# EnricoMiccoli/nodal

Hardware: AMD Instinct MI355X
Metric: circuits_per_sec (higher is better)
Workload: dtype f64; 1 GPU; cfg3: grid(1000) 1e6 nodes, sparse CSR path; n=999999, nnz=4995995, parallelism=one GPU

## Files before the change

nodal_amd/csrc/knobs.h:

```cpp
#pragma once
#include <stdint.h>
#include <stdlib.h>

#include <optional>

namespace knob {

struct Present {
    const char *name;
    bool now() const { return getenv(name) != nullptr; }
};
struct OnUnless0 {
    const char *name;
    bool now() const { const char *e = getenv(name); return !(e && atoi(e) == 0); }
};
struct OffUnlessNon0 {
    const char *name;
    bool now() const { const char *e = getenv(name); return e && atoi(e) != 0; }
};
struct OnIfSet0 {
    const char *name;
    bool now() const { const char *e = getenv(name); return e != nullptr && atoi(e) == 0; }
};
struct Level {
// ... 71 lines not shown
inline constexpr Int64 LOWDEG_MIN{"NODAL_LOWDEG_MIN", 32};
inline constexpr Present SPARSE_FORCE_DIRECT{"NODAL_SPARSE_FORCE_DIRECT"};
inline constexpr Present SPARSE_CHILD_DIRECT{"NODAL_SPARSE_CHILD_DIRECT"};
inline constexpr OnUnless0 SAGG{"NODAL_SAGG"};
inline constexpr OnUnless0 SA_REUSE{"NODAL_SA_REUSE"};
inline constexpr OnUnless0 SA_FORK{"NODAL_SA_FORK"};
inline constexpr Double SA_SPREAD{"NODAL_SA_SPREAD", 16.0};
inline constexpr Double SA_SHARE{"NODAL_SA_SHARE", 0.9};
inline constexpr IntIfSet SA_MIS{"NODAL_SA_MIS"};
inline constexpr Text SA_OMEGA_P{"NODAL_SA_OMEGA_P"};
inline constexpr Double SA_PADSLACK{"NODAL_SA_PADSLACK", 1.3};
inline constexpr OnUnless0 SA_D16{"NODAL_SA_D16"};
inline constexpr Int SA_GG{"NODAL_SA_GG", 40};
inline constexpr Int64 SA_GCAP{"NODAL_SA_GCAP", 16384};
inline constexpr Int SA_GSEG{"NODAL_SA_GSEG", 4};
inline constexpr Text SA_NU{"NODAL_SA_NU"};
inline constexpr Int SA_KCYCLE{"NODAL_SA_KCYCLE", 1};
inline constexpr Int SA_KLEVELS{"NODAL_SA_KLEVELS", 1};
inline constexpr OnUnless0 SA_KFREEZE{"NODAL_SA_KFREEZE"};
inline constexpr OnUnless0 SA_FUSE_DIR{"NODAL_SA_FUSE_DIR"};
inline constexpr OffUnlessNon0 SA_GRAPH{"NODAL_SA_GRAPH"};
inline constexpr Text SA_FOLD_POST{"NODAL_SA_FOLD_POST"};
inline constexpr OffUnlessNon0 SA_FOLD_CHECK{"NODAL_SA_FOLD_CHECK"};
inline constexpr OnUnless0 SA_TAIL_DENSE{"NODAL_SA_TAIL_DENSE"};
inline constexpr OffUnlessNon0 SA_TAIL_CHECK{"NODAL_SA_TAIL_CHECK"};
inline constexpr Int SA_TAIL_NU{"NODAL_SA_TAIL_NU", 3};
inline constexpr Present TAIL_PROBE{"NODAL_TAIL_PROBE"};
inline constexpr IntIfSet AMG_PASSES0{"NODAL_AMG_PASSES0"};
inline constexpr IntIfSet AMG_PASSES1{"NODAL_AMG_PASSES1"};
inline constexpr IntIfSet AMG_SWEEPS0{"NODAL_AMG_SWEEPS0"};
// ... 32 lines not shown
```

nodal_amd/csrc/sagg.hip:

```cpp
#include <hip/hip_ext.h>

#include <atomic>
#include <type_traits>

#include "group.h"

int grounded_flags(nodal_ctx *h, uint8_t *flags_dev);

namespace {

using grp::TB;
constexpr int PW = 4;
constexpr int ACAP = 64;
constexpr int RCAP = 96;
constexpr int RCAP_SMALL = 512;
constexpr int RCAP_SMALL_ROWS = 16384;
inline int rcap_for(int64_t nc) { return nc <= RCAP_SMALL_ROWS ? RCAP_SMALL : RCAP; }
constexpr int W0_MAX = 32;
constexpr int COARSEST = 64;
constexpr int MAX_LEVELS = 12;
constexpr int MIS_ROUNDS = 6;
constexpr int TAIL_MAX_N = 1024;
constexpr int TAIL_LEVELS = 6;
constexpr int TAIL_LDS_BUDGET = 150 * 1024;
// ... 99 lines not shown
    bool dense_coarsest = true;
    DevBuf tail_stamps, tail_image, apcol, apval, aplen, bstat;
    DevBuf tail_op;
    bool tail_dense = false;
    DevBuf mvec;
    hipEvent_t ev_copy = nullptr;
    hipStream_t aux = nullptr;
    hipEvent_t ev_fork = nullptr, ev_join = nullptr, ev_flags = nullptr;
    bool aux_pending = false;
    bool aux_tried = false;
    bool want_flags = false;
    int flags_levels = 0;
    DevBuf stats, coarse_inv, mis_t, mis_m, mis_flag, mis_id, agg1, keys, rstart, cursor, lists;
    TailDesc td;
    uint64_t *host_stats = nullptr;
    bool sym_valid = false;
    uint64_t sym_epoch = 0;
    int64_t sym_n = 0, sym_nnz = 0;
    bool sym_general = false, sym_check = false;
    int32_t sym_floating = 0;
    hipGraph_t it_graph = nullptr;
    hipGraphExec_t it_exec = nullptr;
    uint64_t it_key = 0;
    bool refreshed = false;
    int last_iters = 0;
    int hint_iters = 0;
    int64_t hint_n = 0, hint_nnz = 0;
    int mblock_iters = 0;
    int64_t mblock_n = 0;
    unsigned long long sym_stats[MAX_LEVELS * ST_COUNT] = {0};
// ... 26 lines not shown
        tail_op.release();
        mvec.release();
        tail_stamps.release();
        bstat.release();
        apcol.release();
        apval.release();
        aplen.release();
        DevBuf *b[] = {&stats, &coarse_inv, &mis_t, &mis_m, &mis_flag, &mis_id, &agg1, &keys, &rstart, &cursor, &lists};
        for (DevBuf *x : b) x->release();
        if (host_stats) (void)hipHostFree(host_stats);
    }
};


constexpr int BSTAT_MAX = 65536;
__global__ __launch_bounds__(1024) void reduce_bstat(int nblocks, const uint32_t *__restrict__ bstat,
                                                     unsigned long long *__restrict__ stats, int slot_max,
                                                     int slot_sum) {
    __shared__ unsigned int s_max;
    __shared__ unsigned long long s_sum;
    if (threadIdx.x == 0) { s_max = 0; s_sum = 0; }
    __syncthreads();
    unsigned int m = 0;
    unsigned long long t = 0;
    for (int i = threadIdx.x; i < nblocks; i += 1024) {
        m = max(m, bstat[i]);
        t += bstat[BSTAT_MAX + i];
    }
    atomicMax(&s_max, m);
    atomicAdd(&s_sum, t);
    __syncthreads();
    if (threadIdx.x == 0) {
        if (slot_max >= 0) stats[slot_max] = s_max;
        if (slot_sum >= 0) stats[slot_sum] = s_sum;
    }
}

__global__ __launch_bounds__(TB) void row_stats(int64_t n, const int32_t *__restrict__ indptr,
                                                const int32_t *__restrict__ indices,
                                                const double *__restrict__ data, double share, double spread,
                                                bool general, unsigned long long *__restrict__ stats,
                                                uint32_t *__restrict__ bstat) {
    int32_t mlen = 0;
    uint32_t graded = 0, bad = 0, far = 0;
    for (int64_t i = (int64_t)xcd_block() * TB + threadIdx.x; i < n; i += (int64_t)gridDim.x * TB) {
        const int32_t e0 = indptr[i], e1 = indptr[i + 1];
        mlen = max(mlen, e1 - e0);
        double d = 0.0, mx = 0.0, mn = 1e300;
        for (int32_t e = e0; e < e1; ++e) {
            const double v = data[e];
            const int64_t dc = (int64_t)indices[e] - i;
            if (dc > 32767 || dc < -32767) far = 1;
            if (indices[e] == (int32_t)i) d = v;
            else if (v != 0.0) {
                mx = fmax(mx, fabs(v));
                mn = fmin(mn, fabs(v));
                if (v > 0.0 && !general) bad = 1;
            }
        }
        if (!(d > 0.0)) bad = 1;
        graded += (d > 0.0 && (mx > share * d || mx > spread * mn)) ? 1u : 0u;
    }
    __shared__ unsigned int s_len, s_graded, s_bad;
    if (threadIdx.x == 0) s_len = s_graded = s_bad = 0;
    __syncthreads();
    atomicMax(&s_len, (unsigned)mlen);
    if (graded) atomicAdd(&s_graded, graded);
    if (bad) atomicOr(&s_bad, 1u);
    if (far) atomicOr(&s_bad, 2u);
    __syncthreads();
    if (threadIdx.x == 0) {
        bstat[blockIdx.x] = s_len;
        bstat[BSTAT_MAX + blockIdx.x] = s_graded;
        if (s_bad & 1u) atomicOr(&stats[ST_BADDIAG], 1ull);
        if (s_bad & 2u) stats[ST_FARCOL] = 1ull;
    }
}

__global__ __launch_bounds__(TB) void csr_to_ell(int64_t n, int64_t ld, const int32_t *__restrict__ indptr,
                                                 const int32_t *__restrict__ indices,
                                                 const double *__restrict__ data, int32_t *__restrict__ col,
                                                 double *__restrict__ val, float *__restrict__ valf,
                                                 int32_t *__restrict__ len, double *__restrict__ dinv, int32_t wpad,
                                                 int16_t *__restrict__ dcol) {
    for (int64_t i = (int64_t)xcd_block() * TB + threadIdx.x; i < n; i += (int64_t)gridDim.x * TB) {
        const int32_t e0 = indptr[i], e1 = indptr[i + 1];
        double d = 1.0;
        for (int32_t e = e0; e < e1; ++e) {
            const int32_t c = indices[e];
            const double v = data[e];
            col[(int64_t)(e - e0) * ld + i] = c;
            if (dcol) dcol[(int64_t)(e - e0) * ld + i] = (int16_t)(c - (int32_t)i);
            val[(int64_t)(e - e0) * ld + i] = v;
            valf[(int64_t)(e - e0) * ld + i] = (float)v;
            if (c == (int32_t)i) d = v;
        }
        for (int32_t s = e1 - e0; s < wpad; ++s) {
            col[(int64_t)s * ld + i] = (int32_t)i;
            if (dcol) dcol[(int64_t)s * ld + i] = 0;
// ... 188 lines not shown
                for (int u = 0; u < NB; ++u) {
                    if (s0 + u >= l || c[u] == (int32_t)i || aj[u] < 0) continue;
                    if (w[u] > bw) { bw = w[u]; a = aj[u]; }
                }
            };
            if (l <= 5) batch(std::integral_constant<int, 5>{}, 0);
            else for (int32_t s0 = 0; s0 < l; s0 += 8) batch(std::integral_constant<int, 8>{}, s0);
            if (a < 0) stats[ST_UNASSIGNED] = 1;
        }
        agg[i] = a;
    }
}

__global__ __launch_bounds__(TB) void build_P(Ell A, const double *__restrict__ dinv,
                                              const int32_t *__restrict__ agg, int32_t *__restrict__ pcol,
                                              double *__restrict__ pval, float *__restrict__ pvalf, double omega_p) {
    for (int64_t i = (int64_t)xcd_block() * TB + threadIdx.x; i < A.n; i += (int64_t)gridDim.x * TB) {
        int32_t c[PW];
        double v[PW];
#pragma unroll
        for (int k = 0; k < PW; ++k) { c[k] = -1; v[k] = 0.0; }
        const int32_t own = agg[i];
        c[0] = own;
        v[0] = 1.0;
        const double wd = omega_p * dinv[i];
        const int32_t l = A.len[i];
        for (int32_t s = 0; s < l; ++s) {
            const int32_t J = agg[A.col[(int64_t)s * A.ld + i]];
            const double t = -wd * A.val[(int64_t)s * A.ld + i];
            bool placed = false;
#pragma unroll
// ... 30 lines not shown
                                             uint64_t *__restrict__ keys) {
    for (int64_t i = (int64_t)xcd_block() * TB + threadIdx.x; i < n; i += (int64_t)gridDim.x * TB) {
#pragma unroll
        for (int k = 0; k < PW; ++k) {
            const int32_t J = pcol[(int64_t)k * ld + i];
            if (J >= 0) keys[rstart[J] + place[(int64_t)k * ld + i]] = ((uint64_t)i << 2) | (uint64_t)k;
        }
    }
}
__global__ __launch_bounds__(TB) void r_to_ell(int64_t nc, int64_t rld, const uint32_t *__restrict__ rstart,
                                               const uint64_t *__restrict__ keys, int64_t ld,
                                               const double *__restrict__ pval, int32_t *__restrict__ rcol,
                                               double *__restrict__ rval, float *__restrict__ rvalf,
                                               int32_t *__restrict__ rlen,
                                               unsigned long long *__restrict__ stats, uint32_t *__restrict__ bstat,
                                               uint32_t rcap) {
    uint32_t mlen = 0;
    const int sub = threadIdx.x & 7;
    const int64_t rows_per_pass = (int64_t)gridDim.x * (TB / 8);
    for (int64_t I = (int64_t)xcd_block() * (TB / 8) + threadIdx.x / 8; I < nc; I += rows_per_pass) {
        const uint32_t s0 = rstart[I];
        uint32_t l = rstart[I + 1] - s0;
        mlen = l > mlen ? l : mlen;
        if (l > rcap) l = rcap;
        const uint32_t upto = nc <= 4096 ? rcap : ((l + 7u) & ~7u);
        for (uint32_t t = sub; t < upto; t += 8) {
            const int64_t at = ((int64_t)(t >> 3) * rld + I) * 8 + (t & 7);
            if (t < l) {
                const uint64_t key = keys[s0 + t];
                const int64_t i = (int64_t)(key >> 2);
                const double v = pval[(int64_t)(key & 3) * ld + i];
// ... 8 lines not shown
        }
        if (sub == 0) rlen[I] = (int32_t)l;
    }
    if (mlen > rcap) atomicOr(&stats[ST_OVERFLOW], 2ull);
    __shared__ unsigned int s_max;
    if (threadIdx.x == 0) s_max = 0;
    __syncthreads();
#pragma unroll
    for (int off = 32; off > 0; off >>= 1) {
        const uint32_t o = __shfl_down(mlen, off, 64);
        mlen = o > mlen ? o : mlen;
    }
    if ((threadIdx.x & 63) == 0) atomicMax(&s_max, mlen);
    __syncthreads();
    if (threadIdx.x == 0) {
        bstat[blockIdx.x] = s_max;
        bstat[BSTAT_MAX + blockIdx.x] = 0;
    }
}

__global__ __launch_bounds__(TB) void r_refresh(int64_t nc, int64_t rld, const int32_t *__restrict__ rlen,
                                                const int32_t *__restrict__ rcol, int64_t ld,
                                                const int32_t *__restrict__ pcol, const double *__restrict__ pval,
                                                double *__restrict__ rval, float *__restrict__ rvalf) {
    const int sub = threadIdx.x & 7;
    const int64_t rows_per_pass = (int64_t)gridDim.x * (TB / 8);
    for (int64_t I = (int64_t)xcd_block() * (TB / 8) + threadIdx.x / 8; I < nc; I += rows_per_pass) {
        const int32_t l = rlen[I];
        for (int32_t t = sub; t < l; t += 8) {
            const int64_t at = ((int64_t)(t >> 3) * rld + I) * 8 + (t & 7);
            const int64_t i = rcol[at];
            double v = 0.0;
// ... 278 lines not shown
    }
    for (int p = lane + np; p < np + 72; p += 64) lJ[p] = -1;
    __syncthreads();
    return np;
}

template <bool NUMERIC>
__global__ __launch_bounds__(64) void galerkin(int64_t ld, const int32_t *__restrict__ apcol,
                                               const double *__restrict__ apval, const int32_t *__restrict__ aplen,
                                               int64_t nc, int64_t rld, const int32_t *__restrict__ rcol,
                                               const double *__restrict__ rval, const int32_t *__restrict__ rlen,
                                               int64_t cld, int32_t *__restrict__ ccol, double *__restrict__ cval,
                                               float *__restrict__ cvalf,
                                               int32_t *__restrict__ clen, double *__restrict__ cdinv,
                                               unsigned long long *__restrict__ stats, uint32_t *__restrict__ bstat,
                                               int G, int pcap, int maxseg) {
    extern __shared__ __attribute__((aligned(16))) char gsm[];
    int32_t *set = reinterpret_cast<int32_t *>(gsm);
    double *lV = reinterpret_cast<double *>(gsm + 1024);
    int32_t *lJ = reinterpret_cast<int32_t *>(lV + pcap);
    const int lane = threadIdx.x;
    uint32_t my_max = 0, my_nnz = 0, my_flags = 0;
    for (int64_t I = blockIdx.x; I < nc; I += gridDim.x) {
        const int rl = rlen[I];
        const int ngroups = (rl + G - 1) / G;
        int np = 0;
        int total = 0;
        int32_t myJ = 0x7fffffff;
        if constexpr (NUMERIC) {
            total = clen[I];
            if (lane < total) myJ = ccol[(int64_t)lane * cld + I];
// ... 82 lines not shown
            cval[(int64_t)lane * cld + I] = acc;
            cvalf[(int64_t)lane * cld + I] = (float)acc;
            if (myJ == (int32_t)I) {
                if (!(acc > 0.0)) my_flags |= 4u;
                cdinv[I] = acc > 0.0 ? 1.0 / acc : 1.0;
            }
        }
        if (lane == 0) {
            clen[I] = total;
            my_max = (uint32_t)total > my_max ? (uint32_t)total : my_max;
            my_nnz += (uint32_t)total;
        }
        __syncthreads();
    }
    if (lane == 0) {
        bstat[blockIdx.x] = my_max;
        bstat[BSTAT_MAX + blockIdx.x] = my_nnz;
    }
    if (my_flags & 1u) atomicOr(&stats[ST_OVERFLOW], 1ull);
    if (my_flags & 4u) atomicOr(&stats[ST_BADDIAG], 1ull);
}

__global__ __launch_bounds__(256) void coarsest_inverse(Ell A, double *__restrict__ inv,
                                                        unsigned long long *__restrict__ stats) {
    __shared__ double M[COARSEST][2 * COARSEST + 1];
    const int n = (int)A.n;
    for (int t = threadIdx.x; t < n * 2 * n; t += 256) {
        const int r = t / (2 * n), c = t % (2 * n);
        M[r][c] = (c >= n && c - n == r) ? 1.0 : 0.0;
    }
    __syncthreads();
    for (int r = threadIdx.x; r < n; r += 256)
// ... 73 lines not shown

constexpr int SAGG_DECLINED = -3;

int width_class(int maxlen) {
    static const int classes[] = {4, 5, 6, 8, 12, 16, 20, 24, 32};
    for (int c : classes)
        if (maxlen <= c) return c;
    return 0;
}
int choose_wfix(int maxlen, int64_t n, int64_t nnz, int pad_limit) {
    const int c = width_class(maxlen);
    if (c == 0 || c > pad_limit) return 0;
    static const double slack = knob::SA_PADSLACK.now();
    if ((double)c * (double)n <= slack * (double)nnz || n <= 32768) return c;
    return 0;
}

SHierarchy *hierarchy_of(nodal_ctx *h) {
    if (!h->sagg) h->sagg = new SHierarchy();
    return static_cast<SHierarchy *>(h->sagg);
}

struct SolveBufs {
    double *r, *p, *p2, *Ap, *part_rz, *part_zap, *part_rr, *part_pap, *sc;
    cyc_t *z, *x0;
    int g0;
};

template <bool NUMERIC>
int galerkin_product(nodal_ctx *h, SHierarchy *H, int l, hipEvent_t r_ready = nullptr, int phase = 0) {
// ... 27 lines not shown
    }
    if (phase == 1) return NODAL_OK;
    int G = 1024 / apw;
    G = (G < 8 ? 8 : (G > 64 ? 64 : G));
    static const int g_env = knob::SA_GG.now();
    if (g_env >= 8 && g_env <= 64 && apw == 16) G = g_env & ~7;
    const int pcap = G * apw + 72;
    const size_t lds = 1024 + (size_t)pcap * 12;
    static const int64_t gcap = knob::SA_GCAP.now();
    static const int maxseg = knob::SA_GSEG.now();
    const unsigned gg = (unsigned)(nc < gcap ? nc : (gcap < BSTAT_MAX ? gcap : BSTAT_MAX));
    if (r_ready) NODAL_HIP_TRY(h, hipStreamWaitEvent(st, r_ready, 0));
    galerkin<NUMERIC><<<gg, 64, lds, st>>>(
        ld, apcol, apval, aplen, nc, L->rld, L->rcol.as<int32_t>(), L->rval.as<double>(), L->rlen.as<int32_t>(),
        C->ld, C->acol.as<int32_t>(), C->aval.as<double>(), C->avalf.as<float>(), C->alen.as<int32_t>(),
        C->dinv.as<double>(), dstats + (size_t)(l + 1) * ST_COUNT, H->bstat.as<uint32_t>(), G, pcap, maxseg);
    if (!NUMERIC)
        reduce_bstat<<<1, 1024, 0, st>>>((int)gg, H->bstat.as<uint32_t>(), dstats + (size_t)(l + 1) * ST_COUNT,
                                         ST_MAXLEN, ST_NNZ);
    NODAL_HIP_TRY(h, hipGetLastError());
    return NODAL_OK;
}

double omega_p(int level) {
    static double w[2] = {-1.0, -1.0};
    if (w[0] < 0.0) {
        double a = OMEGA_P, b = OMEGA_P_COARSE;
        if (const char *e = knob::SA_OMEGA_P.now()) {
            a = atof(e);
            const char *c = strchr(e, ',');
            b = c ? atof(c + 1) : a;
        }
// ... 72 lines not shown
    static const int mis_rounds = std::min(MIS_ROUNDS, std::max(1, knob::SA_MIS.now().value_or(MIS_ROUNDS)));
    if (n <= MIS_SMALL_MAX && !trace_mis) {
        mis_small<<<1, 1024, 0, st>>>(A, T, M, flag, mis_rounds);
    } else {
        mis_init<<<g, TB, 0, st>>>(n, T);
        for (int r = 0; r < mis_rounds; ++r) {
            mis_max<<<g, TB, 0, st>>>(A, T, M);
            mis_update<<<g, TB, 0, st>>>(A, T, M);
            if (trace_mis) mis_count<<<g, TB, 0, st>>>(n, T, cnt + r + 1);
        }
        mis_flag_roots<<<grid_for(n + 1), TB, 0, st>>>(A, T, flag);
    }
    NODAL_HIP_TRY(h, hipGetLastError());
    NODAL_TRY(scan_exclusive_u32(h, flag, id, n + 1, reinterpret_cast<uint32_t *>(dstats + (size_t)l * ST_COUNT + ST_NC),
                                 scan_tmp));
    NODAL_HIP_TRY(h, hipMemcpyAsync(hs, dstats, (size_t)MAX_LEVELS * ST_COUNT * 8, hipMemcpyDeviceToHost, st));
    unsigned long long hcnt[MIS_ROUNDS + 1] = {0};
    if (trace_mis) NODAL_HIP_TRY(h, hipMemcpyAsync(hcnt, cnt, sizeof hcnt, hipMemcpyDeviceToHost, st));
    if (!H->ev_copy) NODAL_HIP_TRY(h, hipEventCreateWithFlags(&H->ev_copy, hipEventDisableTiming));
    NODAL_HIP_TRY(h, hipEventRecord(H->ev_copy, st));
    NODAL_HIP_TRY(h, L->pcol.reserve((size_t)PW * ld * 4 + 64));
    NODAL_HIP_TRY(h, L->pval.reserve((size_t)PW * ld * 8 + 64));
    NODAL_HIP_TRY(h, L->pvalf.reserve((size_t)PW * ld * 4 + 64));
    assign_near<<<g, TB, 0, st>>>(A, T, flag, id, H->agg1.as<int32_t>());
    assign_far<<<g, TB, 0, st>>>(A, H->agg1.as<int32_t>(), L->agg.as<int32_t>(), dstats + (size_t)l * ST_COUNT);
    build_P<<<g, TB, 0, st>>>(A, L->dinv.as<double>(), L->agg.as<int32_t>(), L->pcol.as<int32_t>(),
                             L->pval.as<double>(), L->pvalf.as<float>(), omega_p(l));
    NODAL_HIP_TRY(h, hipGetLastError());
    NODAL_WAIT_EVENT(h, H->ev_copy, st);
    if (trace_mis) {
        fprintf(stderr, "[sagg] level %d: undecided after each MIS round:", l);
        for (int r = 1; r <= MIS_ROUNDS; ++r) fprintf(stderr, " %llu", hcnt[r]);
        fprintf(stderr, "\n");
    }
    const int64_t nc = (int64_t)(hs[(size_t)l * ST_COUNT + ST_NC] & 0xffffffffull);
    if (l > 0) {
        const unsigned long long *s = hs + (size_t)l * ST_COUNT;
        L->maxlen = (int32_t)s[ST_MAXLEN];
        L->nnz = (int64_t)s[ST_NNZ];
        A.width = L->maxlen;
        if (s[ST_OVERFLOW] || s[ST_BADDIAG] || hs[(size_t)(l - 1) * ST_COUNT + ST_OVERFLOW] ||
            hs[(size_t)(l - 1) * ST_COUNT + ST_UNASSIGNED]) {
            *declined = true;
            return NODAL_OK;
// ... 36 lines not shown
    C->n = nc;
    C->ld = pad64(nc);
    C->width = ACAP;
    C->nc = 0;
    L->rld = C->ld;
    const int rcap = rcap_for(nc);
    NODAL_HIP_TRY(h, L->rcol.reserve((size_t)rcap * C->ld * 4 + 64));
    NODAL_HIP_TRY(h, L->rval.reserve((size_t)rcap * C->ld * 8 + 64));
    NODAL_HIP_TRY(h, L->rvalf.reserve((size_t)rcap * C->ld * 4 + 64));
    NODAL_HIP_TRY(h, L->rlen.reserve((size_t)C->ld * 4 + 64));
    NODAL_HIP_TRY(h, C->acol.reserve((size_t)ACAP * C->ld * 4 + 64));
    NODAL_HIP_TRY(h, C->aval.reserve((size_t)ACAP * C->ld * 8 + 64));
    NODAL_HIP_TRY(h, C->avalf.reserve((size_t)ACAP * C->ld * 4 + 64));
    NODAL_HIP_TRY(h, C->alen.reserve((size_t)C->ld * 4 + 64));
    NODAL_HIP_TRY(h, C->dinv.reserve((size_t)C->ld * 8 + 64));
    if (forked && H->want_flags) {
        if (l == 0) NODAL_HIP_TRY(h, L->gflag.reserve((size_t)n + 64));
        NODAL_HIP_TRY(h, C->gflag.reserve((size_t)C->n + 64));
    }
    {
        const int apw = L->maxlen <= 6 ? 16 : 64;
        NODAL_HIP_TRY(h, H->apcol.reserve((size_t)apw * ld * 4 + 64));
        NODAL_HIP_TRY(h, H->apval.reserve((size_t)apw * ld * 8 + 64));
        NODAL_HIP_TRY(h, H->aplen.reserve((size_t)ld * 4 + 64));
        L->fold = false;
        L->fold_want = fold_wanted(l, n);
        L->wslots = apw;
        if (L->fold_want) {
            NODAL_HIP_TRY(h, L->wcol.reserve((size_t)apw * ld * 4 + 64));
            NODAL_HIP_TRY(h, L->wval.reserve((size_t)apw * ld * 4 + 64));
            NODAL_HIP_TRY(h, L->wlen.reserve((size_t)ld * 4 + 64));
        }
    }
    hipStream_t main_st = h->stream;
// ... 2 lines not shown
        hipStream_t keep;
        ~StreamGuard() { h->stream = keep; }
    } guard{h, main_st};
    if (forked) {
        NODAL_HIP_TRY(h, hipEventRecord(H->ev_fork, main_st));
        NODAL_HIP_TRY(h, hipStreamWaitEvent(H->aux, H->ev_fork, 0));
        H->aux_pending = true;
        NODAL_TRY(galerkin_product<false>(h, H, l, nullptr, 1));
        h->stream = H->aux;
        st = H->aux;
    }
    char *rs = H->rstart.as<char>();
    uint32_t *rstart = reinterpret_cast<uint32_t *>(rs);
    void *scan_tmp2 = rs + a4 + 256;
    uint32_t *place = reinterpret_cast<uint32_t *>(rs + a4 + 256 + scan2);
    NODAL_HIP_TRY(h, hipMemsetAsync(rs, 0, a4 + 256, st));
    r_count<<<g, TB, 0, st>>>(n, ld, L->pcol.as<int32_t>(), rstart, place);
    NODAL_HIP_TRY(h, hipGetLastError());
    NODAL_TRY(scan_exclusive_u32(h, rstart, rstart, nc + 1, nullptr, scan_tmp2));
    uint64_t *keys = H->keys.as<uint64_t>();
    r_fill<<<g, TB, 0, st>>>(n, ld, L->pcol.as<int32_t>(), rstart, place, keys);
    r_sort_short<<<grid_for(nc), TB, 0, st>>>(rstart, keys, nc);
    r_sort_medium<<<(unsigned)(nc < 8192 ? nc : 8192), 64, 0, st>>>(rstart, keys, nc);
    NODAL_HIP_TRY(h, hipGetLastError());

    {
        const unsigned gr = grid_for(nc * 8);
        r_to_ell<<<gr, TB, 0, st>>>(nc, L->rld, rstart, keys, ld, L->pval.as<double>(), L->rcol.as<int32_t>(),
                                   L->rval.as<double>(), L->rvalf.as<float>(), L->rlen.as<int32_t>(),
                                   dstats + (size_t)l * ST_COUNT, H->bstat.as<uint32_t>(), (uint32_t)rcap);
        reduce_bstat<<<1, 1024, 0, st>>>((int)gr, H->bstat.as<uint32_t>(), dstats + (size_t)l * ST_COUNT, ST_MAXR, -1);
    }
    if (forked) {
        NODAL_HIP_TRY(h, hipGetLastError());
        NODAL_HIP_TRY(h, hipEventRecord(H->ev_join, H->aux));
        if (H->want_flags && H->flags_levels == l) {
            if (l == 0) NODAL_TRY(grounded_flags(h, L->gflag.as<uint8_t>()));
            NODAL_HIP_TRY(h, hipMemsetAsync(C->gflag.p, 0, ((size_t)C->n + 63) & ~(size_t)63, st));
            flags_up<<<grid_for(n), TB, 0, st>>>(n, L->agg.as<int32_t>(), L->gflag.as<uint8_t>(), C->gflag.as<uint8_t>());
            NODAL_HIP_TRY(h, hipGetLastError());
            NODAL_HIP_TRY(h, hipEventRecord(H->ev_flags, H->aux));
            H->flags_levels = l + 1;
        }
        h->stream = main_st;
        st = main_st;
    }
    NODAL_TRY(galerkin_product<false>(h, H, l, forked ? H->ev_join : nullptr, forked ? 2 : 0));
    if (forked && H->flags_levels != l + 1) H->aux_pending = false;
    return NODAL_OK;
}

const void *tail_kernel(int slots) {
    return slots <= 8 ? reinterpret_cast<const void *>(k_tail<8>)
// ... 252 lines not shown
}

int sagg_refresh(nodal_ctx *h, SHierarchy *H, const int32_t *indptr0, const int32_t *indices0, const double *data0,
                 bool general, bool *ok) {
    *ok = false;
    hipStream_t st = h->stream;
    unsigned long long *dstats = H->stats.as<unsigned long long>();
    unsigned long long *hs = reinterpret_cast<unsigned long long *>(H->host_stats);
    NODAL_HIP_TRY(h, hipMemsetAsync(dstats, 0, (size_t)MAX_LEVELS * ST_COUNT * 8, st));
    SLevel *L0 = H->pool[0];
    const int64_t n0 = L0->n;
    {
        const unsigned gr = grid_for(n0);
        static const double spread = knob::SA_SPREAD.now();
        static const double share = knob::SA_SHARE.now();
        row_stats<<<gr, TB, 0, st>>>(n0, indptr0, indices0, data0, share, spread, general, dstats, H->bstat.as<uint32_t>());
        reduce_bstat<<<1, 1024, 0, st>>>((int)gr, H->bstat.as<uint32_t>(), dstats, ST_MAXLEN, ST_GRADED);
    }
    csr_to_ell<<<grid_for(n0), TB, 0, st>>>(n0, L0->ld, indptr0, indices0, data0, L0->acol.as<int32_t>(),
                                           L0->aval.as<double>(), L0->avalf.as<float>(),
                                           L0->alen.as<int32_t>(), L0->dinv.as<double>(), L0->wfix,
                                           L0->d16 ? L0->adcol.as<int16_t>() : nullptr);
    NODAL_HIP_TRY(h, hipGetLastError());
    for (int l = 0; l + 1 < H->nlev; ++l) {
        SLevel *L = H->pool[l], *C = H->pool[l + 1];
        Ell A = L->A();
        A.width = L->maxlen;
        build_P<<<grid_for(L->n), TB, 0, st>>>(A, L->dinv.as<double>(), L->agg.as<int32_t>(), L->pcol.as<int32_t>(),
                                              L->pval.as<double>(), L->pvalf.as<float>(), omega_p(l));
        const bool forked = H->aux != nullptr && nodal_extra_streams_ok(h) &&
                            knob::SA_FORK.now();
        hipStream_t rst = st;
        if (forked) {
            NODAL_HIP_TRY(h, hipEventRecord(H->ev_fork, st));
            NODAL_HIP_TRY(h, hipStreamWaitEvent(H->aux, H->ev_fork, 0));
            H->aux_pending = true;
            NODAL_TRY(galerkin_product<true>(h, H, l, nullptr, 1));
            rst = H->aux;
        }
        r_refresh<<<grid_for(C->n * 8), TB, 0, rst>>>(C->n, L->rld, L->rlen.as<int32_t>(), L->rcol.as<int32_t>(), L->ld,
                                                     L->pcol.as<int32_t>(), L->pval.as<double>(), L->rval.as<double>(),
                                                     L->rvalf.as<float>());
        NODAL_HIP_TRY(h, hipGetLastError());
        if (forked) NODAL_HIP_TRY(h, hipEventRecord(H->ev_join, H->aux));
// ... 61 lines not shown
            H->refreshed = true;
            H->ready = true;
            *accepted = true;
            if (trace) fprintf(stderr, "[sagg] symbolic setup kept (struct epoch %llu): values refreshed\n",
                               (unsigned long long)h->struct_epoch);
            return NODAL_OK;
        }
        if (trace) fprintf(stderr, "[sagg] the kept hierarchy does not take the new values: full setup\n");
    }
    H->sym_valid = false;
    H->refreshed = false;
    H->want_flags = check_floating;
    H->flags_levels = 0;
    H->last_iters = 0;
    H->drop_graph();
    NODAL_HIP_TRY(h, H->stats.reserve((size_t)MAX_LEVELS * ST_COUNT * 8 + 64));
    if (!H->host_stats)
        NODAL_HIP_TRY(h, hipHostMalloc(reinterpret_cast<void **>(&H->host_stats), (size_t)MAX_LEVELS * ST_COUNT * 8 + 64));
    unsigned long long *dstats = H->stats.as<unsigned long long>();
    unsigned long long *hs = reinterpret_cast<unsigned long long *>(H->host_stats);
    NODAL_HIP_TRY(h, hipMemsetAsync(dstats, 0, (size_t)MAX_LEVELS * ST_COUNT * 8, st));
    NODAL_HIP_TRY(h, H->bstat.reserve((size_t)2 * BSTAT_MAX * 4 + 64));
    {
        const unsigned gr = grid_for(n0);
        static const double spread = knob::SA_SPREAD.now();
        static const double share = knob::SA_SHARE.now();
        row_stats<<<gr, TB, 0, st>>>(n0, indptr0, indices0, data0, share, spread, general, dstats, H->bstat.as<uint32_t>());
        reduce_bstat<<<1, 1024, 0, st>>>((int)gr, H->bstat.as<uint32_t>(), dstats, ST_MAXLEN, ST_GRADED);
    }
    NODAL_HIP_TRY(h, hipGetLastError());
    NODAL_HIP_TRY(h, hipMemcpyAsync(hs, dstats, ST_COUNT * 8, hipMemcpyDeviceToHost, st));
    NODAL_WAIT_STREAM(h, st);
    const int64_t bar = n0 / 100 < 32 ? (n0 / 100 > 0 ? n0 / 100 : 1) : 32;
    if (hs[ST_MAXLEN] > (unsigned long long)W0_MAX || hs[ST_MAXLEN] == 0 || hs[ST_BADDIAG] ||
        (int64_t)hs[ST_GRADED] >= bar) {
        if (trace)
            fprintf(stderr, "[sagg] declined: longest row %llu, graded nodes %llu (bar %lld), M-matrix %s\n",
                    hs[ST_MAXLEN], hs[ST_GRADED], (long long)bar, hs[ST_BADDIAG] ? "no" : "yes");
        return NODAL_OK;
    }
    SLevel *L0 = H->level(0);
    L0->n = n0;
    L0->ld = pad64(n0);
    L0->maxlen = (int32_t)hs[ST_MAXLEN];
    L0->nnz = nnz0;
    L0->wfix = choose_wfix(L0->maxlen, n0, nnz0, 8);
    L0->width = L0->wfix ? L0->wfix : L0->maxlen;
    NODAL_HIP_TRY(h, L0->acol.reserve((size_t)L0->width * L0->ld * 4 + 64));
    NODAL_HIP_TRY(h, L0->aval.reserve((size_t)L0->width * L0->ld * 8 + 64));
    NODAL_HIP_TRY(h, L0->avalf.reserve((size_t)L0->width * L0->ld * 4 + 64));
    NODAL_HIP_TRY(h, L0->alen.reserve((size_t)L0->ld * 4 + 64));
    NODAL_HIP_TRY(h, L0->dinv.reserve((size_t)L0->ld * 8 + 64));
    static const bool d16_env = knob::SA_D16.now();
    L0->d16 = d16_env && hs[ST_FARCOL] == 0;
    if (L0->d16) NODAL_HIP_TRY(h, L0->adcol.reserve((size_t)L0->width * L0->ld * 2 + 64));
    csr_to_ell<<<grid_for(n0), TB, 0, st>>>(n0, L0->ld, indptr0, indices0, data0, L0->acol.as<int32_t>(),
                                           L0->aval.as<double>(), L0->avalf.as<float>(),
                                           L0->alen.as<int32_t>(), L0->dinv.as<double>(), L0->wfix,
                                           L0->d16 ? L0->adcol.as<int16_t>() : nullptr);
    NODAL_HIP_TRY(h, hipGetLastError());

    int l = 0;
    bool diag_last = false;
    for (;; ++l) {
        SLevel *L = H->level(l);
        if (L->n <= COARSEST && l > 0) break;
        if (l + 1 >= MAX_LEVELS) {
            if (trace) fprintf(stderr, "[sagg] declined: more than %d levels\n", MAX_LEVELS);
            return NODAL_OK;
        }
        bool declined = false, stop = false;
        NODAL_TRY(build_level(h, H, l, hs, &declined, &stop));
        if (declined) {
            if (trace)
                fprintf(stderr, "[sagg] declined at level %d (%lld rows): does not coarsen / over a cap / not positive "
// ... 1 lines not shown
                        l, (long long)L->n, hs[(size_t)l * ST_COUNT + ST_OVERFLOW], hs[(size_t)l * ST_COUNT + ST_BADDIAG],
                        l > 0 ? hs[(size_t)(l - 1) * ST_COUNT + ST_OVERFLOW] : 0ull,
                        l > 0 ? hs[(size_t)(l - 1) * ST_COUNT + ST_UNASSIGNED] : 0ull,
                        l > 0 ? hs[(size_t)(l - 1) * ST_COUNT + ST_MAXR] : 0ull);
            return NODAL_OK;
        }
        if (stop) {
            diag_last = true;
            break;
        }
    }
    H->nlev = l + 1;
    SLevel *last = H->level(l);
    last->fold_want = last->fold = false;
    if (H->nlev < 2) return NODAL_OK;
    NODAL_HIP_TRY(h, hipMemcpyAsync(hs, dstats, (size_t)MAX_LEVELS * ST_COUNT * 8, hipMemcpyDeviceToHost, st));
    if (!H->ev_copy) NODAL_HIP_TRY(h, hipEventCreateWithFlags(&H->ev_copy, hipEventDisableTiming));
    NODAL_HIP_TRY(h, hipEventRecord(H->ev_copy, st));
    if (check_floating) {
        if (H->flags_levels == 0) {
            NODAL_HIP_TRY(h, H->level(0)->gflag.reserve((size_t)n0 + 64));
            NODAL_TRY(grounded_flags(h, H->level(0)->gflag.as<uint8_t>()));
        } else {
            NODAL_HIP_TRY(h, hipStreamWaitEvent(st, H->ev_flags, 0));
            H->aux_pending = false;
        }
        for (int k = H->flags_levels; k + 1 < H->nlev; ++k) {
            SLevel *L = H->pool[k], *C = H->pool[k + 1];
            NODAL_HIP_TRY(h, C->gflag.reserve((size_t)C->n + 64));
            NODAL_HIP_TRY(h, hipMemsetAsync(C->gflag.p, 0, ((size_t)C->n + 63) & ~(size_t)63, st));
            flags_up<<<grid_for(L->n), TB, 0, st>>>(L->n, L->agg.as<int32_t>(), L->gflag.as<uint8_t>(),
                                                   C->gflag.as<uint8_t>());
        }
        NODAL_HIP_TRY(h, hipGetLastError());
    }
    NODAL_WAIT_EVENT(h, H->ev_copy, st);
    for (int k = 0; k < H->nlev; ++k) {
        const unsigned long long *s = hs + (size_t)k * ST_COUNT;
        if (k > 0) {
            H->pool[k]->maxlen = (int32_t)s[ST_MAXLEN];
            H->pool[k]->nnz = (int64_t)s[ST_NNZ];
            H->pool[k]->wfix = choose_wfix(H->pool[k]->maxlen, H->pool[k]->n, H->pool[k]->nnz, APAD);
        }
        if (s[ST_OVERFLOW] || (k > 0 && s[ST_BADDIAG]) || s[ST_UNASSIGNED]) {
            if (trace) fprintf(stderr, "[sagg] declined: level %d over a cap / not positive\n", k);
            return NODAL_OK;
        }
    }
    diag_last = last->maxlen <= 1;
    H->dense_coarsest = !diag_last;
    if (H->dense_coarsest) {
        if (last->n > COARSEST) return NODAL_OK;
        NODAL_HIP_TRY(h, H->coarse_inv.reserve((size_t)last->n * last->n * 8 + 64));
        coarsest_inverse<<<1, 256, 0, st>>>(last->A(), H->coarse_inv.as<double>(),
                                            dstats + (size_t)l * ST_COUNT);
        NODAL_HIP_TRY(h, hipGetLastError());
    }
    for (int k = 0; k < H->nlev; ++k) {
        SLevel *L = H->pool[k];
        NODAL_HIP_TRY(h, L->vec.reserve((size_t)V_COUNT * L->ld * 8 + 256));
        NODAL_HIP_TRY(h, L->part.reserve(5 * DOT_BLOCKS * 8 + 512));
    }
    NODAL_TRY(build_tail(h, H, hs));

    if (!check_floating) {
        NODAL_HIP_TRY(h, hipMemcpyAsync(hs, dstats, (size_t)MAX_LEVELS * ST_COUNT * 8, hipMemcpyDeviceToHost, st));
        NODAL_WAIT_STREAM(h, st);
        if (hs[(size_t)l * ST_COUNT + ST_BADDIAG] & 2ull) return NODAL_OK;
    } else {
        uint32_t *fl = reinterpret_cast<uint32_t *>(dstats + (size_t)(MAX_LEVELS - 1) * ST_COUNT + ST_COUNT - 1);
        if (H->dense_coarsest) last_level_floating<<<1, 64, 0, st>>>(last->A(), last->gflag.as<uint8_t>(), fl);
        else any_unflagged<<<grid_for(last->n), TB, 0, st>>>(last->n, last->gflag.as<uint8_t>(), fl);
        NODAL_HIP_TRY(h, hipGetLastError());
        NODAL_HIP_TRY(h, hipMemcpyAsync(hs, dstats, (size_t)MAX_LEVELS * ST_COUNT * 8, hipMemcpyDeviceToHost, st));
        NODAL_WAIT_STREAM(h, st);
        if (hs[(size_t)l * ST_COUNT + ST_BADDIAG] & 2ull) {
            if (trace) fprintf(stderr, "[sagg] declined: coarsest matrix not positive definite\n");
            return NODAL_OK;
        }
        *floating = hs[(size_t)(MAX_LEVELS - 1) * ST_COUNT + ST_COUNT - 1] != 0 ? 1 : 0;
    }
    if (trace) {
        fprintf(stderr, "[sagg] levels (rows/entries/longest row/padded width):");
        for (int k = 0; k < H->nlev; ++k)
            fprintf(stderr, " %lld/%lld/%d/%d", (long long)H->pool[k]->n, (long long)H->pool[k]->nnz,
                    H->pool[k]->maxlen, H->pool[k]->wfix);
        fprintf(stderr, "  tail %d (%d register slots)  coarsest %s\n", H->tail, H->tail >= 0 ? H->td.slots : 0,
                H->dense_coarsest ? "dense" : "diagonal");
    }
    decide_folds(H, hs, trace);
// ... 473 lines not shown
```

Baseline: 164.8 circuits/s.

## Fold setup statistics into per-block atomic partials and drop separate memset and reduce launches

Adds a lean setup mode, on by default, in which row_stats, r_to_ell and galerkin write per-block maxima and sums into 32 striped partial lines through atomics. The host folds those lines after its readback, so the single-block reduce_bstat launches go away. Zeroing of the stats block, the restriction row-start buffer and the coarse ground-flag arrays moves into kernels that already run (row_stats, build_P, r_to_ell, csr_to_ell), which removes several hipMemsetAsync calls. This cuts launch count and serial small kernels in AMG setup, at the cost of more intricate zeroing invariants and a somewhat larger host copy of the stats area.

Result: no change. 163.2 circuits/s (-1.0%).

```diff
diff --git a/nodal_amd/csrc/knobs.h b/nodal_amd/csrc/knobs.h
--- a/nodal_amd/csrc/knobs.h
+++ b/nodal_amd/csrc/knobs.h
@@ -109,6 +109,7 @@
 inline constexpr Int SA_GG{"NODAL_SA_GG", 40};
 inline constexpr Int64 SA_GCAP{"NODAL_SA_GCAP", 16384};
 inline constexpr Int SA_GSEG{"NODAL_SA_GSEG", 4};
+inline constexpr OnUnless0 SA_SETUP_LEAN{"NODAL_SA_SETUP_LEAN"};
 inline constexpr Text SA_NU{"NODAL_SA_NU"};
 inline constexpr Int SA_KCYCLE{"NODAL_SA_KCYCLE", 1};
 inline constexpr Int SA_KLEVELS{"NODAL_SA_KLEVELS", 1};
diff --git a/nodal_amd/csrc/sagg.hip b/nodal_amd/csrc/sagg.hip
--- a/nodal_amd/csrc/sagg.hip
+++ b/nodal_amd/csrc/sagg.hip
@@ -137,6 +137,8 @@
     DevBuf stats, coarse_inv, mis_t, mis_m, mis_flag, mis_id, agg1, keys, rstart, cursor, lists;
     TailDesc td;
     uint64_t *host_stats = nullptr;
+    bool stats_primed = false;
+    unsigned long long row0[4] = {0, 0, 0, 0};
     bool sym_valid = false;
     uint64_t sym_epoch = 0;
     int64_t sym_n = 0, sym_nnz = 0;
@@ -193,6 +195,23 @@
 
 
 constexpr int BSTAT_MAX = 65536;
+constexpr int SPART = 32;
+constexpr int SPART_LINE = 32;
+constexpr int SPART_BASE = 128;
+enum { SP_MAX = 0, SP_SUM = 1, SP_MAXR = 2 };
+constexpr size_t STATS_BLOCK_BYTES = (size_t)MAX_LEVELS * ST_COUNT * 8;
+constexpr size_t STATS_WORDS = SPART_BASE + (size_t)MAX_LEVELS * SPART * SPART_LINE;
+static_assert(STATS_BLOCK_BYTES <= SPART_BASE * 8, "the partial lines begin behind the statistics block");
+inline size_t stats_bytes_upto(int level) { return (SPART_BASE + (size_t)(level + 1) * SPART * SPART_LINE) * 8; }
+__host__ __device__ inline unsigned long long *stats_partials(unsigned long long *stats, int level) {
+    return stats + SPART_BASE + (size_t)level * SPART * SPART_LINE;
+}
+__device__ __forceinline__ void stat_partial(unsigned long long *__restrict__ part, int slot_max, uint32_t mx, int slot_sum,
+                                             uint32_t sum) {
+    unsigned long long *line = part + (size_t)(blockIdx.x % SPART) * SPART_LINE;
+    if (mx) atomicMax(&line[slot_max], (unsigned long long)mx);
+    if (slot_sum >= 0 && sum) atomicAdd(&line[slot_sum], (unsigned long long)sum);
+}
 __global__ __launch_bounds__(1024) void reduce_bstat(int nblocks, const uint32_t *__restrict__ bstat,
                                                      unsigned long long *__restrict__ stats, int slot_max,
                                                      int slot_sum) {
@@ -219,7 +238,13 @@
                                                 const int32_t *__restrict__ indices,
                                                 const double *__restrict__ data, double share, double spread,
                                                 bool general, unsigned long long *__restrict__ stats,
-                                                uint32_t *__restrict__ bstat) {
+                                                uint32_t *__restrict__ bstat, bool lean) {
+    if (lean)
+        for (size_t w = (size_t)blockIdx.x * TB + threadIdx.x; w < STATS_WORDS; w += (size_t)gridDim.x * TB) {
+            const bool mine = w == ST_BADDIAG || w == ST_FARCOL ||
+                              (w >= SPART_BASE && w < SPART_BASE + SPART * SPART_LINE && (w % SPART_LINE) <= SP_SUM);
+            if (!mine) stats[w] = 0ull;
+        }
     int32_t mlen = 0;
     uint32_t graded = 0, bad = 0, far = 0;
     for (int64_t i = (int64_t)xcd_block() * TB + threadIdx.x; i < n; i += (int64_t)gridDim.x * TB) {
@@ -249,8 +274,12 @@
     if (far) atomicOr(&s_bad, 2u);
     __syncthreads();
     if (threadIdx.x == 0) {
-        bstat[blockIdx.x] = s_len;
-        bstat[BSTAT_MAX + blockIdx.x] = s_graded;
+        if (lean) {
+            stat_partial(stats_partials(stats, 0), SP_MAX, s_len, SP_SUM, s_graded);
+        } else {
+            bstat[blockIdx.x] = s_len;
+            bstat[BSTAT_MAX + blockIdx.x] = s_graded;
+        }
         if (s_bad & 1u) atomicOr(&stats[ST_BADDIAG], 1ull);
         if (s_bad & 2u) stats[ST_FARCOL] = 1ull;
     }
@@ -261,7 +290,14 @@
                                                  const double *__restrict__ data, int32_t *__restrict__ col,
                                                  double *__restrict__ val, float *__restrict__ valf,
                                                  int32_t *__restrict__ len, double *__restrict__ dinv, int32_t wpad,
-                                                 int16_t *__restrict__ dcol) {
+                                                 int16_t *__restrict__ dcol,
+                                                 unsigned long long *__restrict__ clear_stats) {
+    if (clear_stats && blockIdx.x == 0 && threadIdx.x < SPART) {
+        unsigned long long *line = stats_partials(clear_stats, 0) + (size_t)threadIdx.x * SPART_LINE;
+        line[SP_MAX] = 0ull;
+        line[SP_SUM] = 0ull;
+        if (threadIdx.x == 0) clear_stats[ST_BADDIAG] = clear_stats[ST_FARCOL] = 0ull;
+    }
     for (int64_t i = (int64_t)xcd_block() * TB + threadIdx.x; i < n; i += (int64_t)gridDim.x * TB) {
         const int32_t e0 = indptr[i], e1 = indptr[i + 1];
         double d = 1.0;
@@ -480,7 +516,9 @@
 
 __global__ __launch_bounds__(TB) void build_P(Ell A, const double *__restrict__ dinv,
                                               const int32_t *__restrict__ agg, int32_t *__restrict__ pcol,
-                                              double *__restrict__ pval, float *__restrict__ pvalf, double omega_p) {
+                                              double *__restrict__ pval, float *__restrict__ pvalf, double omega_p,
+                                              uint32_t *__restrict__ zero, int64_t nzero) {
+    for (int64_t w = (int64_t)blockIdx.x * TB + threadIdx.x; w < nzero; w += (int64_t)gridDim.x * TB) zero[w] = 0u;
     for (int64_t i = (int64_t)xcd_block() * TB + threadIdx.x; i < A.n; i += (int64_t)gridDim.x * TB) {
         int32_t c[PW];
         double v[PW];
@@ -541,7 +579,10 @@
                                                double *__restrict__ rval, float *__restrict__ rvalf,
                                                int32_t *__restrict__ rlen,
                                                unsigned long long *__restrict__ stats, uint32_t *__restrict__ bstat,
-                                               uint32_t rcap) {
+                                               uint32_t rcap, unsigned long long *__restrict__ part,
+                                               uint8_t *__restrict__ gzero, int64_t ngzero) {
+    for (int64_t w = (int64_t)blockIdx.x * TB + threadIdx.x; w < ngzero; w += (int64_t)gridDim.x * TB)
+        reinterpret_cast<uint32_t *>(gzero)[w] = 0u;
     uint32_t mlen = 0;
     const int sub = threadIdx.x & 7;
     const int64_t rows_per_pass = (int64_t)gridDim.x * (TB / 8);
@@ -580,8 +621,12 @@
     if ((threadIdx.x & 63) == 0) atomicMax(&s_max, mlen);
     __syncthreads();
     if (threadIdx.x == 0) {
-        bstat[blockIdx.x] = s_max;
-        bstat[BSTAT_MAX + blockIdx.x] = 0;
+        if (part) {
+            stat_partial(part, SP_MAXR, s_max, -1, 0u);
+        } else {
+            bstat[blockIdx.x] = s_max;
+            bstat[BSTAT_MAX + blockIdx.x] = 0;
+        }
     }
 }
 
@@ -890,7 +935,7 @@
                                                float *__restrict__ cvalf,
                                                int32_t *__restrict__ clen, double *__restrict__ cdinv,
                                                unsigned long long *__restrict__ stats, uint32_t *__restrict__ bstat,
-                                               int G, int pcap, int maxseg) {
+                                               int G, int pcap, int maxseg, unsigned long long *__restrict__ part) {
     extern __shared__ __attribute__((aligned(16))) char gsm[];
     int32_t *set = reinterpret_cast<int32_t *>(gsm);
     double *lV = reinterpret_cast<double *>(gsm + 1024);
@@ -1003,8 +1048,12 @@
         __syncthreads();
     }
     if (lane == 0) {
-        bstat[blockIdx.x] = my_max;
-        bstat[BSTAT_MAX + blockIdx.x] = my_nnz;
+        if (part) {
+            stat_partial(part, SP_MAX, my_max, SP_SUM, my_nnz);
+        } else {
+            bstat[blockIdx.x] = my_max;
+            bstat[BSTAT_MAX + blockIdx.x] = my_nnz;
+        }
     }
     if (my_flags & 1u) atomicOr(&stats[ST_OVERFLOW], 1ull);
     if (my_flags & 4u) atomicOr(&stats[ST_BADDIAG], 1ull);
@@ -1108,6 +1157,37 @@
     static const double slack = knob::SA_PADSLACK.now();
     if ((double)c * (double)n <= slack * (double)nnz || n <= 32768) return c;
     return 0;
+}
+
+bool setup_lean() {
+    static const bool on = knob::SA_SETUP_LEAN.now();
+    return on;
+}
+hipError_t stats_copy(SHierarchy *H, int upto, hipStream_t st) {
+    const size_t bytes = setup_lean() ? stats_bytes_upto(upto < MAX_LEVELS ? upto : MAX_LEVELS - 1) : STATS_BLOCK_BYTES;
+    return hipMemcpyAsync(H->host_stats, H->stats.p, bytes, hipMemcpyDeviceToHost, st);
+}
+void stats_fold(SHierarchy *H, int upto, bool first = false) {
+    if (!setup_lean()) return;
+    unsigned long long *hs = reinterpret_cast<unsigned long long *>(H->host_stats);
+    for (int k = 0; k <= upto && k < MAX_LEVELS; ++k) {
+        const unsigned long long *part = stats_partials(hs, k);
+        unsigned long long mx = 0, sum = 0, mr = 0;
+        for (int j = 0; j < SPART; ++j) {
+            mx = std::max(mx, part[(size_t)j * SPART_LINE + SP_MAX]);
+            sum += part[(size_t)j * SPART_LINE + SP_SUM];
+            mr = std::max(mr, part[(size_t)j * SPART_LINE + SP_MAXR]);
+        }
+        unsigned long long *s = hs + (size_t)k * ST_COUNT;
+        s[ST_MAXLEN] = mx;
+        s[k == 0 ? ST_GRADED : ST_NNZ] = sum;
+        s[ST_MAXR] = mr;
+    }
+    if (first) {
+        H->row0[0] = hs[ST_MAXLEN]; H->row0[1] = hs[ST_GRADED]; H->row0[2] = hs[ST_BADDIAG]; H->row0[3] = hs[ST_FARCOL];
+    } else {
+        hs[ST_MAXLEN] = H->row0[0]; hs[ST_GRADED] = H->row0[1]; hs[ST_BADDIAG] = H->row0[2]; hs[ST_FARCOL] = H->row0[3];
+    }
 }
 
 SHierarchy *hierarchy_of(nodal_ctx *h) {
@@ -1165,8 +1245,9 @@
     galerkin<NUMERIC><<<gg, 64, lds, st>>>(
         ld, apcol, apval, aplen, nc, L->rld, L->rcol.as<int32_t>(), L->rval.as<double>(), L->rlen.as<int32_t>(),
         C->ld, C->acol.as<int32_t>(), C->aval.as<double>(), C->avalf.as<float>(), C->alen.as<int32_t>(),
-        C->dinv.as<double>(), dstats + (size_t)(l + 1) * ST_COUNT, H->bstat.as<uint32_t>(), G, pcap, maxseg);
-    if (!NUMERIC)
+        C->dinv.as<double>(), dstats + (size_t)(l + 1) * ST_COUNT, H->bstat.as<uint32_t>(), G, pcap, maxseg,
+        !NUMERIC && setup_lean() ? stats_partials(dstats, l + 1) : nullptr);
+    if (!NUMERIC && !setup_lean())
         reduce_bstat<<<1, 1024, 0, st>>>((int)gg, H->bstat.as<uint32_t>(), dstats + (size_t)(l + 1) * ST_COUNT,
                                          ST_MAXLEN, ST_NNZ);
     NODAL_HIP_TRY(h, hipGetLastError());
@@ -1269,7 +1350,7 @@
     NODAL_HIP_TRY(h, hipGetLastError());
     NODAL_TRY(scan_exclusive_u32(h, flag, id, n + 1, reinterpret_cast<uint32_t *>(dstats + (size_t)l * ST_COUNT + ST_NC),
                                  scan_tmp));
-    NODAL_HIP_TRY(h, hipMemcpyAsync(hs, dstats, (size_t)MAX_LEVELS * ST_COUNT * 8, hipMemcpyDeviceToHost, st));
+    NODAL_HIP_TRY(h, stats_copy(H, l, st));
     unsigned long long hcnt[MIS_ROUNDS + 1] = {0};
     if (trace_mis) NODAL_HIP_TRY(h, hipMemcpyAsync(hcnt, cnt, sizeof hcnt, hipMemcpyDeviceToHost, st));
     if (!H->ev_copy) NODAL_HIP_TRY(h, hipEventCreateWithFlags(&H->ev_copy, hipEventDisableTiming));
@@ -1277,12 +1358,17 @@
     NODAL_HIP_TRY(h, L->pcol.reserve((size_t)PW * ld * 4 + 64));
     NODAL_HIP_TRY(h, L->pval.reserve((size_t)PW * ld * 8 + 64));
     NODAL_HIP_TRY(h, L->pvalf.reserve((size_t)PW * ld * 4 + 64));
+    const bool lean = setup_lean();
+    const size_t rzero = lean ? align256((size_t)(n + 1) * 4) + 256 : 0;
+    if (lean) NODAL_HIP_TRY(h, H->rstart.reserve(rzero + align256(scan_tmp_bytes(n + 1)) + (size_t)PW * ld * 4 + 64));
     assign_near<<<g, TB, 0, st>>>(A, T, flag, id, H->agg1.as<int32_t>());
     assign_far<<<g, TB, 0, st>>>(A, H->agg1.as<int32_t>(), L->agg.as<int32_t>(), dstats + (size_t)l * ST_COUNT);
     build_P<<<g, TB, 0, st>>>(A, L->dinv.as<double>(), L->agg.as<int32_t>(), L->pcol.as<int32_t>(),
-                             L->pval.as<double>(), L->pvalf.as<float>(), omega_p(l));
+                             L->pval.as<double>(), L->pvalf.as<float>(), omega_p(l),
+                             lean ? H->rstart.as<uint32_t>() : nullptr, (int64_t)(rzero / 4));
     NODAL_HIP_TRY(h, hipGetLastError());
     NODAL_WAIT_EVENT(h, H->ev_copy, st);
+    stats_fold(H, l);
     if (trace_mis) {
         fprintf(stderr, "[sagg] level %d: undecided after each MIS round:", l);
         for (int r = 1; r <= MIS_ROUNDS; ++r) fprintf(stderr, " %llu", hcnt[r]);
@@ -1349,10 +1435,8 @@
     NODAL_HIP_TRY(h, C->avalf.reserve((size_t)ACAP * C->ld * 4 + 64));
     NODAL_HIP_TRY(h, C->alen.reserve((size_t)C->ld * 4 + 64));
     NODAL_HIP_TRY(h, C->dinv.reserve((size_t)C->ld * 8 + 64));
-    if (forked && H->want_flags) {
-        if (l == 0) NODAL_HIP_TRY(h, L->gflag.reserve((size_t)n + 64));
-        NODAL_HIP_TRY(h, C->gflag.reserve((size_t)C->n + 64));
-    }
+    if (forked && H->want_flags && l == 0) NODAL_HIP_TRY(h, L->gflag.reserve((size_t)n + 64));
+    if ((forked || lean) && H->want_flags) NODAL_HIP_TRY(h, C->gflag.reserve((size_t)C->n + 64));
     {
         const int apw = L->maxlen <= 6 ? 16 : 64;
         NODAL_HIP_TRY(h, H->apcol.reserve((size_t)apw * ld * 4 + 64));
@@ -1385,7 +1469,7 @@
     uint32_t *rstart = reinterpret_cast<uint32_t *>(rs);
     void *scan_tmp2 = rs + a4 + 256;
     uint32_t *place = reinterpret_cast<uint32_t *>(rs + a4 + 256 + scan2);
-    NODAL_HIP_TRY(h, hipMemsetAsync(rs, 0, a4 + 256, st));
+    if (!lean) NODAL_HIP_TRY(h, hipMemsetAsync(rs, 0, a4 + 256, st));
     r_count<<<g, TB, 0, st>>>(n, ld, L->pcol.as<int32_t>(), rstart, place);
     NODAL_HIP_TRY(h, hipGetLastError());
     NODAL_TRY(scan_exclusive_u32(h, rstart, rstart, nc + 1, nullptr, scan_tmp2));
@@ -1399,15 +1483,19 @@
         const unsigned gr = grid_for(nc * 8);
         r_to_ell<<<gr, TB, 0, st>>>(nc, L->rld, rstart, keys, ld, L->pval.as<double>(), L->rcol.as<int32_t>(),
                                    L->rval.as<double>(), L->rvalf.as<float>(), L->rlen.as<int32_t>(),
-                                   dstats + (size_t)l * ST_COUNT, H->bstat.as<uint32_t>(), (uint32_t)rcap);
-        reduce_bstat<<<1, 1024, 0, st>>>((int)gr, H->bstat.as<uint32_t>(), dstats + (size_t)l * ST_COUNT, ST_MAXR, -1);
+                                   dstats + (size_t)l * ST_COUNT, H->bstat.as<uint32_t>(), (uint32_t)rcap,
+                                   lean ? stats_partials(dstats, l) : nullptr,
+                                   lean && H->want_flags ? C->gflag.as<uint8_t>() : nullptr,
+                                   lean && H->want_flags ? pad64(C->n) / 4 : 0);
+        if (!lean)
+            reduce_bstat<<<1, 1024, 0, st>>>((int)gr, H->bstat.as<uint32_t>(), dstats + (size_t)l * ST_COUNT, ST_MAXR, -1);
     }
     if (forked) {
         NODAL_HIP_TRY(h, hipGetLastError());
         NODAL_HIP_TRY(h, hipEventRecord(H->ev_join, H->aux));
         if (H->want_flags && H->flags_levels == l) {
             if (l == 0) NODAL_TRY(grounded_flags(h, L->gflag.as<uint8_t>()));
-            NODAL_HIP_TRY(h, hipMemsetAsync(C->gflag.p, 0, ((size_t)C->n + 63) & ~(size_t)63, st));
+            if (!lean) NODAL_HIP_TRY(h, hipMemsetAsync(C->gflag.p, 0, ((size_t)C->n + 63) & ~(size_t)63, st));
             flags_up<<<grid_for(n), TB, 0, st>>>(n, L->agg.as<int32_t>(), L->gflag.as<uint8_t>(), C->gflag.as<uint8_t>());
             NODAL_HIP_TRY(h, hipGetLastError());
             NODAL_HIP_TRY(h, hipEventRecord(H->ev_flags, H->aux));
@@ -1690,20 +1778,22 @@
         const unsigned gr = grid_for(n0);
         static const double spread = knob::SA_SPREAD.now();
         static const double share = knob::SA_SHARE.now();
-        row_stats<<<gr, TB, 0, st>>>(n0, indptr0, indices0, data0, share, spread, general, dstats, H->bstat.as<uint32_t>());
+        H->stats_primed = false;
+        row_stats<<<gr, TB, 0, st>>>(n0, indptr0, indices0, data0, share, spread, general, dstats, H->bstat.as<uint32_t>(),
+                                    false);
         reduce_bstat<<<1, 1024, 0, st>>>((int)gr, H->bstat.as<uint32_t>(), dstats, ST_MAXLEN, ST_GRADED);
     }
     csr_to_ell<<<grid_for(n0), TB, 0, st>>>(n0, L0->ld, indptr0, indices0, data0, L0->acol.as<int32_t>(),
                                            L0->aval.as<double>(), L0->avalf.as<float>(),
                                            L0->alen.as<int32_t>(), L0->dinv.as<double>(), L0->wfix,
-                                           L0->d16 ? L0->adcol.as<int16_t>() : nullptr);
+                                           L0->d16 ? L0->adcol.as<int16_t>() : nullptr, nullptr);
     NODAL_HIP_TRY(h, hipGetLastError());
     for (int l = 0; l + 1 < H->nlev; ++l) {
         SLevel *L = H->pool[l], *C = H->pool[l + 1];
         Ell A = L->A();
         A.width = L->maxlen;
         build_P<<<grid_for(L->n), TB, 0, st>>>(A, L->dinv.as<double>(), L->agg.as<int32_t>(), L->pcol.as<int32_t>(),
-                                              L->pval.as<double>(), L->pvalf.as<float>(), omega_p(l));
+                                              L->pval.as<double>(), L->pvalf.as<float>(), omega_p(l), nullptr, 0);
         const bool forked = H->aux != nullptr && nodal_extra_streams_ok(h) &&
                             knob::SA_FORK.now();
         hipStream_t rst = st;
@@ -1795,23 +1885,29 @@
     H->flags_levels = 0;
     H->last_iters = 0;
     H->drop_graph();
-    NODAL_HIP_TRY(h, H->stats.reserve((size_t)MAX_LEVELS * ST_COUNT * 8 + 64));
+    const bool lean = setup_lean();
+    NODAL_HIP_TRY(h, H->stats.reserve(STATS_WORDS * 8 + 64));
     if (!H->host_stats)
-        NODAL_HIP_TRY(h, hipHostMalloc(reinterpret_cast<void **>(&H->host_stats), (size_t)MAX_LEVELS * ST_COUNT * 8 + 64));
+        NODAL_HIP_TRY(h, hipHostMalloc(reinterpret_cast<void **>(&H->host_stats), STATS_WORDS * 8 + 64));
     unsigned long long *dstats = H->stats.as<unsigned long long>();
     unsigned long long *hs = reinterpret_cast<unsigned long long *>(H->host_stats);
-    NODAL_HIP_TRY(h, hipMemsetAsync(dstats, 0, (size_t)MAX_LEVELS * ST_COUNT * 8, st));
+    if (!lean) NODAL_HIP_TRY(h, hipMemsetAsync(dstats, 0, STATS_BLOCK_BYTES, st));
+    else if (!H->stats_primed) NODAL_HIP_TRY(h, hipMemsetAsync(dstats, 0, STATS_WORDS * 8, st));
+    H->stats_primed = false;
     NODAL_HIP_TRY(h, H->bstat.reserve((size_t)2 * BSTAT_MAX * 4 + 64));
     {
         const unsigned gr = grid_for(n0);
         static const double spread = knob::SA_SPREAD.now();
         static const double share = knob::SA_SHARE.now();
-        row_stats<<<gr, TB, 0, st>>>(n0, indptr0, indices0, data0, share, spread, general, dstats, H->bstat.as<uint32_t>());
-        reduce_bstat<<<1, 1024, 0, st>>>((int)gr, H->bstat.as<uint32_t>(), dstats, ST_MAXLEN, ST_GRADED);
+        row_stats<<<gr, TB, 0, st>>>(n0, indptr0, indices0, data0, share, spread, general, dstats, H->bstat.as<uint32_t>(),
+                                    lean);
+        if (!lean) reduce_bstat<<<1, 1024, 0, st>>>((int)gr, H->bstat.as<uint32_t>(), dstats, ST_MAXLEN, ST_GRADED);
     }
     NODAL_HIP_TRY(h, hipGetLastError());
-    NODAL_HIP_TRY(h, hipMemcpyAsync(hs, dstats, ST_COUNT * 8, hipMemcpyDeviceToHost, st));
+    if (lean) NODAL_HIP_TRY(h, stats_copy(H, 0, st));
+    else NODAL_HIP_TRY(h, hipMemcpyAsync(hs, dstats, ST_COUNT * 8, hipMemcpyDeviceToHost, st));
     NODAL_WAIT_STREAM(h, st);
+    stats_fold(H, 0, true);
     const int64_t bar = n0 / 100 < 32 ? (n0 / 100 > 0 ? n0 / 100 : 1) : 32;
     if (hs[ST_MAXLEN] > (unsigned long long)W0_MAX || hs[ST_MAXLEN] == 0 || hs[ST_BADDIAG] ||
         (int64_t)hs[ST_GRADED] >= bar) {
@@ -1838,8 +1934,9 @@
     csr_to_ell<<<grid_for(n0), TB, 0, st>>>(n0, L0->ld, indptr0, indices0, data0, L0->acol.as<int32_t>(),
                                            L0->aval.as<double>(), L0->avalf.as<float>(),
                                            L0->alen.as<int32_t>(), L0->dinv.as<double>(), L0->wfix,
-                                           L0->d16 ? L0->adcol.as<int16_t>() : nullptr);
+                                           L0->d16 ? L0->adcol.as<int16_t>() : nullptr, lean ? dstats : nullptr);
     NODAL_HIP_TRY(h, hipGetLastError());
+    H->stats_primed = lean;
 
     int l = 0;
     bool diag_last = false;
@@ -1871,7 +1968,7 @@
     SLevel *last = H->level(l);
     last->fold_want = last->fold = false;
     if (H->nlev < 2) return NODAL_OK;
-    NODAL_HIP_TRY(h, hipMemcpyAsync(hs, dstats, (size_t)MAX_LEVELS * ST_COUNT * 8, hipMemcpyDeviceToHost, st));
+    NODAL_HIP_TRY(h, stats_copy(H, l, st));
     if (!H->ev_copy) NODAL_HIP_TRY(h, hipEventCreateWithFlags(&H->ev_copy, hipEventDisableTiming));
     NODAL_HIP_TRY(h, hipEventRecord(H->ev_copy, st));
     if (check_floating) {
@@ -1885,13 +1982,14 @@
         for (int k = H->flags_levels; k + 1 < H->nlev; ++k) {
             SLevel *L = H->pool[k], *C = H->pool[k + 1];
             NODAL_HIP_TRY(h, C->gflag.reserve((size_t)C->n + 64));
-            NODAL_HIP_TRY(h, hipMemsetAsync(C->gflag.p, 0, ((size_t)C->n + 63) & ~(size_t)63, st));
+            if (!lean) NODAL_HIP_TRY(h, hipMemsetAsync(C->gflag.p, 0, ((size_t)C->n + 63) & ~(size_t)63, st));
             flags_up<<<grid_for(L->n), TB, 0, st>>>(L->n, L->agg.as<int32_t>(), L->gflag.as<uint8_t>(),
                                                    C->gflag.as<uint8_t>());
         }
         NODAL_HIP_TRY(h, hipGetLastError());
     }
     NODAL_WAIT_EVENT(h, H->ev_copy, st);
+    stats_fold(H, l);
     for (int k = 0; k < H->nlev; ++k) {
         const unsigned long long *s = hs + (size_t)k * ST_COUNT;
         if (k > 0) {
@@ -1921,16 +2019,18 @@
     NODAL_TRY(build_tail(h, H, hs));
 
     if (!check_floating) {
-        NODAL_HIP_TRY(h, hipMemcpyAsync(hs, dstats, (size_t)MAX_LEVELS * ST_COUNT * 8, hipMemcpyDeviceToHost, st));
+        NODAL_HIP_TRY(h, stats_copy(H, l, st));
         NODAL_WAIT_STREAM(h, st);
+        stats_fold(H, l);
         if (hs[(size_t)l * ST_COUNT + ST_BADDIAG] & 2ull) return NODAL_OK;
     } else {
         uint32_t *fl = reinterpret_cast<uint32_t *>(dstats + (size_t)(MAX_LEVELS - 1) * ST_COUNT + ST_COUNT - 1);
         if (H->dense_coarsest) last_level_floating<<<1, 64, 0, st>>>(last->A(), last->gflag.as<uint8_t>(), fl);
         else any_unflagged<<<grid_for(last->n), TB, 0, st>>>(last->n, last->gflag.as<uint8_t>(), fl);
         NODAL_HIP_TRY(h, hipGetLastError());
-        NODAL_HIP_TRY(h, hipMemcpyAsync(hs, dstats, (size_t)MAX_LEVELS * ST_COUNT * 8, hipMemcpyDeviceToHost, st));
+        NODAL_HIP_TRY(h, stats_copy(H, l, st));
         NODAL_WAIT_STREAM(h, st);
+        stats_fold(H, l);
         if (hs[(size_t)l * ST_COUNT + ST_BADDIAG] & 2ull) {
             if (trace) fprintf(stderr, "[sagg] declined: coarsest matrix not positive definite\n");
             return NODAL_OK;
```
